# medhini/audio-video-textures

Measured on AMD Instinct MI355X. Metric: clip-windows/sec encoded + N×N transition build, N=4096; HBM GB/s achieved, higher is better.
Workload: dtype f16x3

## Files before the change

### audio-video-textures_amd/_lib.py

```python
import ctypes as C
import os
import re

_HERE = os.path.dirname(os.path.abspath(__file__))
LIB_PATH = os.environ.get("AVT_HIP_LIB") or os.path.join(_HERE, "libavt_hip.so")
HEADER_PATH = os.path.join(os.path.dirname(_HERE), "include", "avt.h")


class AvtError(RuntimeError):
    pass


_SCALARS = {"int": C.c_int, "int64_t": C.c_int64, "float": C.c_float, "double": C.c_double, "size_t": C.c_size_t}
_DECL = re.compile(r"\b(int|int64_t|const\s+char\s*\*)\s*\b(avt_[a-z0-9_]+)\s*\(([^()]*)\)\s*;")


def _ctype(decl, name):
    words = [w for w in decl.replace("*", " * ").replace("[", " [").split() if w != "const"]
    if any(w[0] in "*[" for w in words):
        return C.c_char_p if words[0] == "char" else C.c_void_p
    if not 1 <= len(words) <= 2 or words[0] not in _SCALARS:
        raise AvtError("include/avt.h: %s has a parameter `%s` whose type this binding does not know" % (name, decl.strip()))
    return _SCALARS[words[0]]

# ... 31 lines not shown

def _bind(fn):
    fn.restype, fn.argtypes = _ABI[fn.__name__]
    return fn


def lib():
    global _lib
    if _lib is None:
        if not os.path.exists(LIB_PATH):
            raise AvtError(
                "HIP extension not built: %s is missing. Run `make -C %s` (needs hipcc); "
                "there is no CPU fallback for the hot path." % (LIB_PATH, os.path.join(_HERE, "csrc")))
        handle = C.CDLL(LIB_PATH)
        for name in _ABI:
            if not hasattr(handle, name):
                raise AvtError("libavt_hip.so does not export %s: rebuild with `make -C %s`" % (name, os.path.join(_HERE, "csrc")))
            _bind(getattr(handle, name))
        if handle.avt_abi_version() != ABI_VERSION:
            raise AvtError("libavt_hip.so ABI version %d, expected %d: rebuild with `make -C %s`"
                           % (handle.avt_abi_version(), ABI_VERSION, os.path.join(_HERE, "csrc")))
        if os.environ.get("AVT_SMALL_TILE", "") == "0":
            handle.avt_conv_x3_set_small_tile(0)
        if os.environ.get("AVT_WGRAD_ROUNDS", "") == "0":
            handle.avt_wgrad_x3_set_xl(7)
        _lib = handle
    return _lib


def _failure(what, status):
    msg = lib().avt_last_error()
    return AvtError("%s failed (%d): %s" % (what, status, msg.decode() if msg else "?"))


def check(status, what):
    if status != 0:
        raise _failure(what, status)


def _errcheck(status, fn, args):
    if status != 0:
        raise _failure(fn.__name__, status)
    return status


class _Checked:
# ... 12 lines not shown
```

### audio-video-textures_amd/csrc/conv_args.h

```cpp
#pragma once
#include "avt_common.h"

namespace {

constexpr unsigned kOob = 0xFFFFFFF0u;
constexpr int kMaxTabSteps = 128;

constexpr int LSTR = 144;
constexpr int BK = 64;

struct FastDiv {
  uint32_t d, magic, shift;
};
inline FastDiv make_fastdiv(uint32_t d) {
  FastDiv f{d, 0u, 0u};
  if (d > 1) {
    uint32_t s = 0;
    while ((1ull << s) < d) ++s;
    f.magic = (uint32_t)((((1ull << 32) * ((1ull << s) - d)) / d) + 1);
    f.shift = s - 1;
  }
  return f;
}
__device__ __forceinline__ uint32_t fastdiv(uint32_t n, const FastDiv& f) {
  const uint32_t t = __umulhi(n, f.magic);
  const uint32_t q = (t + ((n - t) >> 1)) >> f.shift;
  return f.d == 1 ? n : q;
}

struct ConvArgs {
  const uint16_t* in;
  const uint16_t* wt;
  const float* bias;
  const uint16_t* res;
  uint16_t* out;
  const int2* ktab;
  int T, H, W;
  int To, Ho, Wo;
  int Cout, K;
  int KT, KH, KW, st, sh, sw, pt, ph, pw;
  int ldi, ldo, ldr;
  int relu;
  int M;
  int nk;
  int tiles_n, nblk;
  FastDiv dWo, dHo, dTo;
  FastDiv dCpt, dKHW, dKW;
  FastDiv dNT;
  int tapinner;
  unsigned in_bytes, wt_bytes;
  int pointwise;
  const uint16_t* wfrag;
  int nup;
  int wblk;
  unsigned wf_bytes;
  int ors, oH, oW;
  const uint16_t* in_lo;
  const uint16_t* wt_lo;
  const uint16_t* res_lo;
  uint16_t* out_lo;
  const float* wscale;
  float odiv;
  int cf_ofs;
  double* stat_part;
  int stat_groups, stat_mg, stat_tpg;
  int stat_c;
  const float* bst_x;
  const float* bst_mean;
  const float* bst_invstd;
  const float* bst_gamma;
  const float* bst_beta;
  const uint8_t* bst_mask;
  int bst_relu;
};

struct BstCoef {
  float mu[8], sc[8], be[8];
};
__device__ __forceinline__ void bst_load(const ConvArgs& a, int group, int n, BstCoef& k) {
  const int C = a.stat_c;
#pragma unroll
  for (int e = 0; e < 8; ++e) {
    const int c = (n + e) % C;
    k.mu[e] = a.bst_mean[(size_t)group * C + c];
    k.sc[e] = a.bst_invstd[(size_t)group * C + c] * a.bst_gamma[c];
    k.be[e] = a.bst_beta ? a.bst_beta[c] : 0.0f;
  }
}
__device__ __forceinline__ void bst_apply(const ConvArgs& a, const BstCoef& k, const float* xv, unsigned bits, float* x, float* s, float* q) {
  const bool by_bits = a.bst_relu != 0 && a.bst_mask != nullptr, by_x = a.bst_relu != 0 && a.bst_mask == nullptr;
  const unsigned mbits = by_bits ? bits : 0xFFu;
#pragma unroll
  for (int e = 0; e < 8; ++e) {
    const float xc = xv[e] - k.mu[e];
    const float act = by_x ? xc * k.sc[e] + k.be[e] : 1.0f;
    const float sel = (((mbits >> e) & 1u) != 0u && act > 0.0f) ? 1.0f : 0.0f;
// ... 98 lines not shown
  AVT_REQUIRE(M < (1ll << 31) && (int64_t)g.batch * g.t * g.h * g.w * g.ldi < (1ll << 31) - 64 && M * (int64_t)g.ldo < (1ll << 62) &&
                  (int64_t)g.cout * a.K < (1ll << 31) - 64,
              "%s: tensor too large for 32-bit offsets", who);
  a.in_bytes = (unsigned)((int64_t)g.batch * g.t * g.h * g.w * g.ldi * 2);
  a.wt_bytes = (unsigned)((int64_t)g.cout * a.K * 2);
  a.M = (int)M;
  a.nk = (a.K + BK - 1) / BK;
  a.pointwise = (g.kt == 1 && g.kh == 1 && g.kw == 1 && g.st == 1 && g.sh == 1 && g.sw == 1 && g.pt == 0 && g.ph == 0 && g.pw == 0 &&
                 a.To == g.t && a.Ho == g.h && a.Wo == g.w) ? 1 : 0;
  a.dWo = make_fastdiv((uint32_t)a.Wo);
  a.dHo = make_fastdiv((uint32_t)a.Ho);
  a.dTo = make_fastdiv((uint32_t)a.To);
  const bool remap = g.out_row_stride > 1 || (g.out_h > 0 && g.out_w > 0);
  AVT_REQUIRE(g.out_row_stride >= 1 && (!remap || (!res && g.out_h >= g.out_row_stride * (a.Ho - 1) + 1 &&
                                                   g.out_w >= g.out_row_stride * (a.Wo - 1) + 1)),
              "%s: the remapped rows need an out_h x out_w grid that holds %d x (%d x %d), no residual", who,
              g.out_row_stride, a.Ho, a.Wo);
  AVT_REQUIRE(!remap || (int64_t)g.batch * a.To * g.out_h * g.out_w < (1ll << 31),
              "%s: output buffer too large for 32-bit rows", who);
  a.ors = g.out_row_stride;
  a.oH = remap ? g.out_h : 0;
  a.oW = remap ? g.out_w : 0;
  a.stat_part = nullptr;
  a.odiv = 0.0f;
  a.stat_groups = a.stat_mg = a.stat_tpg = a.stat_c = 0;
  a.bst_x = a.bst_mean = a.bst_invstd = a.bst_gamma = a.bst_beta = nullptr;
  a.bst_mask = nullptr;
  a.bst_relu = 0;
  return AVT_OK;
}

}
```

### audio-video-textures_amd/csrc/conv_x3.hip

```cpp
#include <stdlib.h>

#include <type_traits>

#include "avt_common.h"
#include "conv_args.h"
#include "launch.h"
#include "mfma.h"
#include "split_planes.h"

#ifdef AVT_CONV_STAMP
#define AVT_STAMP_FN avt_debug_stamps_x3
namespace {
#include "../../tools/diag/conv_stamp.h"
}
#ifndef AVT_DBG_CONST
#define AVT_DBG_CONST 0
#endif
#define DBG_SKIP(bit) (((AVT_DBG_CONST) & (bit)) != 0)
#ifdef AVT_STAMP_EPI
#define KSTAMP(i) STAMP(0)
#define EPI_STAMP(i) STAMP(i)
#else
#define KSTAMP(i) STAMP(i)
#define EPI_STAMP(i)
// ... 385 lines not shown
#pragma unroll
      for (int e = 0; e < 8; ++e) {
        red[(tr * 2 + 0) * BN + cc * 8 + e] = st_s[e];
        red[(tr * 2 + 1) * BN + cc * 8 + e] = st_q[e];
      }
      __syncthreads();
      stat_fold_store<BN, 256>(a, red, 256 / CPR, tm, n0, tid);
    }
  }
  STAMP_END();
}

template <bool F16, bool IO32 = false, bool OUT32 = IO32>
__global__ __launch_bounds__(512, 2) void conv_x3_xl_kernel(ConvArgs a) {
  constexpr int BM = 256, BN = 256, NTHR = 512, KB = 32;
  constexpr int MT = 4, NT = 2;
  constexpr int AU = BM / 128, BU = BN / 128;
  constexpr int PL = BM * 64;
  constexpr int STG = 4 * PL;
  constexpr int ESTR = BN * 4 + 16;
  extern __shared__ __attribute__((aligned(16))) char lds[];

  const int swz = avt::xcd_contiguous(blockIdx.x, a.nblk);
  const int tm = swz / a.tiles_n, tn = swz % a.tiles_n;
  const int n0 = tn * BN;
  int m0, m_end;
  if constexpr (IO32) tile_rows(a, tm, BM, m0, m_end);
  else { m0 = tm * BM; m_end = a.M; }
  const int tid = threadIdx.x;
  const int lane = tid & 63, wid = tid >> 6;
  const int wm = wid >> 2, wn = wid & 3;
  const int lr = lane & 31, lh = lane >> 5;
  const int r0 = tid >> 2, c4 = (tid & 3) ^ ((r0 >> 2) & 3);

  int rowoff[AU];
  unsigned rowmask[AU];
#pragma unroll
  for (int u = 0; u < AU; ++u) {
    const int m = m0 + r0 + 128 * u;
    rowoff[u] = 0;
    rowmask[u] = 0u;
    if (m < m_end && a.pointwise) {
      rowoff[u] = m * a.ldi;
      rowmask[u] = 0x010101u;
    } else if (m < m_end) {
      const int t1 = (int)fastdiv((uint32_t)m, a.dWo), wo = m - t1 * a.Wo;
      const int t2 = (int)fastdiv((uint32_t)t1, a.dHo), ho = t1 - t2 * a.Ho;
      const int b = (int)fastdiv((uint32_t)t2, a.dTo), to = t2 - b * a.To;
      const int ti0 = to * a.st - a.pt, hi0 = ho * a.sh - a.ph, wi0 = wo * a.sw - a.pw;
      rowoff[u] = (((b * a.T + ti0) * a.H + hi0) * a.W + wi0) * a.ldi;
      unsigned mask = 0u;
      for (int dt = 0; dt < a.KT; ++dt) mask |= ((unsigned)(ti0 + dt) < (unsigned)a.T ? 1u : 0u) << dt;
      for (int dh = 0; dh < a.KH; ++dh) mask |= ((unsigned)(hi0 + dh) < (unsigned)a.H ? 1u : 0u) << (8 + dh);
      for (int dw = 0; dw < a.KW; ++dw) mask |= ((unsigned)(wi0 + dw) < (unsigned)a.W ? 1u : 0u) << (16 + dw);
      rowmask[u] = mask;
    }
  }
  int wrow[BU];
  unsigned wsel[BU];
#pragma unroll
  for (int u = 0; u < BU; ++u) {
    const int n = n0 + r0 + 128 * u;
    wrow[u] = n < a.Cout ? n * a.K : 0;
    wsel[u] = n < a.Cout ? 0xFFFFFFFFu : 0u;
  }

  f32x16 acc[NT][MT];
#pragma unroll
  for (int i = 0; i < NT; ++i)
#pragma unroll
    for (int j = 0; j < MT; ++j)
#pragma unroll
      for (int r = 0; r < 16; ++r) acc[i][j][r] = 0.0f;
  const __amdgpu_buffer_rsrc_t rih = avt::buffer_rsrc(a.in, a.in_bytes);
  const __amdgpu_buffer_rsrc_t ril = avt::buffer_rsrc(a.in_lo, a.in_bytes);
  const __amdgpu_buffer_rsrc_t rwh = avt::buffer_rsrc(a.wt, a.wt_bytes);
  const __amdgpu_buffer_rsrc_t rwl = avt::buffer_rsrc(a.wt_lo, a.wt_bytes);
  int2* ltab = reinterpret_cast<int2*>(lds + 2 * STG);
  for (int i = tid; i < a.nk * 8; i += NTHR) ltab[i] = a.ktab[i];
  const int nk32 = (a.K + KB - 1) / KB;

  unsigned aoffs[AU], boffs[BU];
  auto gtab = [&](int kt) -> int2 { return ltab[kt * 4 + c4]; };
  auto gcalc = [&](int kt, int2 e) {
    const unsigned ebits = (unsigned)e.y;
#pragma unroll
    for (int u = 0; u < AU; ++u) {
      const unsigned sel = ((rowmask[u] & ebits) == ebits) ? 0xFFFFFFFFu : 0u;
      aoffs[u] = (((unsigned)(rowoff[u] + e.x) * (IO32 ? 4u : 2u)) & sel) | (kOob & ~sel);
    }
    const unsigned ksel = ~(unsigned)(e.y >> 31);
    const unsigned kc2 = (unsigned)((kt * 4 + c4) * 16);
#pragma unroll
    for (int u = 0; u < BU; ++u) {
      const unsigned sel = ksel & wsel[u];
      boffs[u] = (((unsigned)wrow[u] * 2u + kc2) & sel) | (kOob & ~sel);
      if (a.wblk) boffs[u] = (((unsigned)(kt * a.Cout + n0 + r0 + 128 * u) * 64u + (unsigned)c4 * 16u) & sel) | (kOob & ~sel);
    }
  };
  auto gprep = [&](int kt) { gcalc(kt, gtab(kt)); };
  constexpr int NPIECE = 2 * (AU + BU);
  typedef __attribute__((address_space(3))) void* lds_ptr;
  const int wrow0 = wid * 16 * 64;
  auto gpiece = [&](int p, char* st) {
    if (p < 2 * AU) {
      const int u = p >> 1;
      __builtin_amdgcn_raw_ptr_buffer_load_lds((p & 1) ? ril : rih, (lds_ptr)(st + (p & 1) * PL + wrow0 + u * 128 * 64), 16,
                                               (int)aoffs[u], 0, 0, 0);
    } else {
      const int u = (p - 2 * AU) >> 1;
      __builtin_amdgcn_raw_ptr_buffer_load_lds((p & 1) ? rwl : rwh, (lds_ptr)(st + (2 + (p & 1)) * PL + wrow0 + u * 128 * 64), 16,
                                               (int)boffs[u], 0, 0, 0);
    }
  };
  i32x4 ra[IO32 ? AU : 1][2];
  auto aload = [&]() {
    if constexpr (IO32) {
#pragma unroll
      for (int u = 0; u < AU; ++u) {
        const unsigned o2 = aoffs[u] == kOob ? kOob : aoffs[u] + 16u;
        ra[u][0] = __builtin_amdgcn_raw_buffer_load_b128(rih, (int)aoffs[u], 0, 0);
        ra[u][1] = __builtin_amdgcn_raw_buffer_load_b128(rih, (int)o2, 0, 0);
      }
// ... 40 lines not shown
    for (int i = 0; i < NT; ++i)
#pragma unroll
      for (int j = 0; j < MT; ++j) {
        acc[i][j] = mfma32<F16>(f.wl[i], f.ah[j], acc[i][j]);
        acc[i][j] = mfma32<F16>(f.wh[i], f.al[j], acc[i][j]);
        acc[i][j] = mfma32<F16>(f.wh[i], f.ah[j], acc[i][j]);
        const int pc = g0 + i * MT + j + (IO32 ? 2 * AU : 0);
        if (more && pc < NPIECE) gpiece(pc, nst);
        __builtin_amdgcn_sched_barrier(0);
      }
  };

  float* cfl = reinterpret_cast<float*>(lds + a.cf_ofs);
  {
    const int n = n0 + (tid & 255);
    float v = tid < 256 ? 0.0f : 1.0f;
    if (n < a.Cout) {
      if (tid < 256) { if (a.bias) v = a.bias[n]; } else if (a.wscale) v = a.wscale[n];
    }
    cfl[tid] = v;
  }
  __syncthreads();
  STAMP_BEGIN();
  gprep(0);
  if constexpr (IO32) {
    aload();
#pragma unroll
    for (int p = 2 * AU; p < NPIECE; ++p) gpiece(p, lds);
    asm volatile("s_waitcnt vmcnt(0)" ::: "memory");
    astore(lds);
  } else {
#pragma unroll
    for (int p = 0; p < NPIECE; ++p) gpiece(p, lds);
    asm volatile("s_waitcnt vmcnt(0)" ::: "memory");
  }
  __syncthreads();
  STAMP(0);
  if constexpr (IO32) {
    for (int kt = 0; kt < nk32; ++kt) {
      const bool more = kt + 1 < nk32;
      char* cur = lds + (kt & 1) * STG;
      char* nst = lds + ((kt + 1) & 1) * STG;
      int2 e = make_int2(0, 0);
      if (more) e = gtab(kt + 1);
      Frags f;
      fload(f, cur, 0);
      if (more) {
        gcalc(kt + 1, e);
        aload();
      }
      __builtin_amdgcn_sched_barrier(0);
      fmul(f, 0, more, nst);
      fload(f, cur, 1);
      __builtin_amdgcn_sched_barrier(0);
      fmul(f, NPIECE, false, nst);
      asm volatile("s_waitcnt vmcnt(0)" ::: "memory");
      if (more) astore(nst);
      __syncthreads();
    }
  } else {
    Frags f0, f1;
    fload(f0, lds, 0);
    if (nk32 > 1) gprep(1);
    fload(f1, lds, 1);
    __builtin_amdgcn_sched_barrier(0);
    fmul(f0, 0, nk32 > 1, lds + STG);
    asm volatile("s_waitcnt vmcnt(0) lgkmcnt(0)" ::: "memory");
    __syncthreads();
    for (int kt = 1; kt < nk32; ++kt) {
      const bool more = kt + 1 < nk32;
      char* cur = lds + (kt & 1) * STG;
      char* nst = lds + ((kt + 1) & 1) * STG;
      int2 e = make_int2(0, 0);
      if (more) e = gtab(kt + 1);
      fload(f0, cur, 0);
      if (more) gcalc(kt + 1, e);
      __builtin_amdgcn_sched_barrier(0);
      fmul(f1, 0, more, nst);
      KSTAMP(1);
      fload(f1, cur, 1);
      __builtin_amdgcn_sched_barrier(0);
      fmul(f0, NPIECE, false, nst);
      KSTAMP(2);
      asm volatile("s_waitcnt vmcnt(0) lgkmcnt(0)" ::: "memory");
      KSTAMP(3);
      __syncthreads();
      KSTAMP(4);
    }
    fmul(f1, NPIECE, false, lds);
  }

  constexpr int SR = 64;
  constexpr int CPR = BN / 8;
  constexpr int EU = (SR * CPR) / NTHR;
  constexpr int EBUF = SR * ESTR;
  static_assert(2 * EBUF <= 2 * STG + kMaxTabSteps * 64, "two staging buffers fit the operand stages + the table area");
  const bool has_res = !OUT32 && a.res != nullptr;
  auto stage_slab = [&](auto half, int pass) {
    constexpr int H = decltype(half)::value;
    char* eb = lds + (pass & 1) * EBUF;
#pragma unroll
    for (int i = 0; i < NT; ++i)
#pragma unroll
      for (int g = 0; g < 4; ++g) {
        const int nl = wn * 64 + i * 32 + 8 * g + 4 * lh;
        const float4 bv = *reinterpret_cast<const float4*>(cfl + nl);
        const float4 sv = *reinterpret_cast<const float4*>(cfl + 256 + nl);
#pragma unroll
        for (int jj = 0; jj < 2; ++jj) {
          const int j = 2 * H + jj;
          float4 v;
          v.x = acc[i][j][4 * g + 0] * sv.x + bv.x;
          v.y = acc[i][j][4 * g + 1] * sv.y + bv.y;
          v.z = acc[i][j][4 * g + 2] * sv.z + bv.z;
          v.w = acc[i][j][4 * g + 3] * sv.w + bv.w;
          const int rl = jj * 32 + lr;
          *reinterpret_cast<float4*>(eb + rl * ESTR + nl * 4) = v;
        }
      }
  };
  KSTAMP(5);
  if (wm == 0) stage_slab(std::integral_constant<int, 0>{}, 0);
  __syncthreads();
  EPI_STAMP(1);
  float st_s[IO32 ? 8 : 1], st_q[IO32 ? 8 : 1];
  if constexpr (IO32) {
#pragma unroll
    for (int e = 0; e < 8; ++e) st_s[e] = st_q[e] = 0.0f;
  }
#pragma unroll 1
  for (int pass = 0; pass < 4; ++pass) {
    const char* eb = lds + (pass & 1) * EBUF;
    uint4 rrh[EU], rrl[EU];
    if (has_res) {
#pragma unroll
      for (int u = 0; u < EU; ++u) {
        const int c = tid + NTHR * u;
        const int m = m0 + pass * SR + c / CPR, n = n0 + (c % CPR) * 8;
        const bool ok = m < m_end && n < a.Cout;
        rrh[u] = ok ? *reinterpret_cast<const uint4*>(a.res + (int64_t)m * a.ldr + n) : make_uint4(0u, 0u, 0u, 0u);
        rrl[u] = ok ? *reinterpret_cast<const uint4*>(a.res_lo + (int64_t)m * a.ldr + n) : make_uint4(0u, 0u, 0u, 0u);
      }
    }
    if constexpr (IO32) {
      if (a.res) {
#pragma unroll
        for (int u = 0; u < EU; ++u) {
          const int c = tid + NTHR * u;
          const int m = m0 + pass * SR + c / CPR, n = n0 + (c % CPR) * 8;
          const bool ok = m < m_end && n < a.Cout;
          const float* rf = reinterpret_cast<const float*>(a.res) + (int64_t)m * a.ldr + n;
          rrh[u] = ok ? *reinterpret_cast<const uint4*>(rf) : make_uint4(0u, 0u, 0u, 0u);
          rrl[u] = ok ? *reinterpret_cast<const uint4*>(rf + 4) : make_uint4(0u, 0u, 0u, 0u);
        }
      }
    }
    if (pass + 1 < 4 && wm == ((pass + 1) >> 1)) {
      if ((pass + 1) & 1) stage_slab(std::integral_constant<int, 1>{}, pass + 1);
      else stage_slab(std::integral_constant<int, 0>{}, pass + 1);
    }
    EPI_STAMP(2);
#pragma unroll
    for (int u = 0; u < EU; ++u) {
      const int c = tid + NTHR * u;
      const int row = c / CPR, cc = c % CPR;
      const int m = m0 + pass * SR + row, n = n0 + cc * 8;
      if (m < m_end && n < a.Cout) {
        const float4 v0 = *reinterpret_cast<const float4*>(eb + row * ESTR + cc * 32);
        const float4 v1 = *reinterpret_cast<const float4*>(eb + row * ESTR + cc * 32 + 16);
        float x[8] = {v0.x, v0.y, v0.z, v0.w, v1.x, v1.y, v1.z, v1.w};
        if (has_res) {
          const uint32_t* ph = reinterpret_cast<const uint32_t*>(&rrh[u]);
          const uint32_t* pl = reinterpret_cast<const uint32_t*>(&rrl[u]);
#pragma unroll
          for (int e = 0; e < 4; ++e) {
            const avt::f32x2 r = avt::join2<F16>(ph[e], pl[e]);
            x[2 * e] += r.x;
            x[2 * e + 1] += r.y;
          }
        }
        if (a.relu == 1) {
#pragma unroll
          for (int e = 0; e < 8; ++e) x[e] = avt::relu_keep_nan(x[e]);
        } else if (a.relu == 2) {
#pragma unroll
          for (int e = 0; e < 8; ++e) x[e] = fmaxf(x[e], 0.1f * x[e]);
        }
        const int64_t o = (int64_t)out_row(a, m) * a.ldo + n;
        if constexpr (OUT32) {
// ... 29 lines not shown
    EPI_STAMP(3);
    __syncthreads();
    EPI_STAMP(4);
  }
  if constexpr (IO32) {
    if (a.stat_part) {
      float* red = reinterpret_cast<float*>(lds);
      const int tr = tid / CPR, cc = tid % CPR;
#pragma unroll
      for (int e = 0; e < 8; ++e) {
        red[(tr * 2 + 0) * BN + cc * 8 + e] = st_s[e];
        red[(tr * 2 + 1) * BN + cc * 8 + e] = st_q[e];
      }
      __syncthreads();
      stat_fold_store<BN, NTHR>(a, red, NTHR / CPR, tm, n0, tid);
    }
  }
  STAMP_END();
}

template <bool F16, bool IO32 = false, bool OUT32 = IO32>
int launch_x3_xl(ConvArgs& a, hipStream_t st) {
  if (a.stat_part) a.stat_tpg = (a.stat_mg + 255) / 256;
  const int tiles_m = a.stat_part ? a.stat_groups * a.stat_tpg : (a.M + 255) / 256;
  a.tiles_n = (a.Cout + 255) / 256;
  a.nblk = tiles_m * a.tiles_n;
  constexpr int lds_bytes = 2 * 4 * 256 * 64 + kMaxTabSteps * 64 + 2 * 256 * 4;
  a.cf_ofs = lds_bytes - 2 * 256 * 4;
  return avt::launch<conv_x3_xl_kernel<F16, IO32, OUT32>>("avt_conv3d_igemm_x3", dim3((unsigned)a.nblk), dim3(512), lds_bytes, lds_bytes,
                                                          st, a);
}

template <int BM, int BN, int WTM, bool F16, bool IO32 = false, bool BST = false>
int launch_x3(ConvArgs& a, hipStream_t st) {
  if (a.stat_part) a.stat_tpg = (a.stat_mg + BM - 1) / BM;
  const int tiles_m = a.stat_part ? a.stat_groups * a.stat_tpg : (a.M + BM - 1) / BM;
  a.tiles_n = (a.Cout + BN - 1) / BN;
  a.nblk = tiles_m * a.tiles_n;
  constexpr int epi_bytes = BM * (BN * 4 + 16);
  constexpr int opnd_max = 2 * (BM + BN) * LSTR + kMaxTabSteps * 64;
  constexpr int lds_max = (opnd_max > epi_bytes ? opnd_max : epi_bytes) + 2 * BN * 4;
  const int tab_bytes = (a.nk <= kMaxTabSteps ? a.nk : 0) * 64;
  int lds_bytes = 2 * (BM + BN) * LSTR + tab_bytes;
  if (lds_bytes < epi_bytes) lds_bytes = epi_bytes;
  a.cf_ofs = lds_bytes;
  lds_bytes += 2 * BN * 4;
  return avt::launch<conv_x3_kernel<BM, BN, WTM, F16, IO32, BST>>("avt_conv3d_igemm_x3", dim3((unsigned)a.nblk), dim3(256), lds_max,
                                                                  lds_bytes, st, a);
}

template <bool F16, bool IO32 = false, bool BST = false>
int launch_x3_by_cout(ConvArgs& a, hipStream_t st, bool small = false) {
  if (a.Cout <= 32) return launch_x3<128, 32, 32, F16, IO32, BST>(a, st);
  if (a.Cout <= 64) return launch_x3<128, 64, 64, F16, IO32, BST>(a, st);
  if constexpr (IO32) {
    if (small) return launch_x3<64, 128, 32, F16, IO32, BST>(a, st);
  }
  return launch_x3<128, 128, 64, F16, IO32, BST>(a, st);
}

struct X3Planes {
  const void *in_hi, *in_lo, *wt_hi, *wt_lo;
  const float* bias;
  const void *res_hi, *res_lo;
  void *out_hi, *out_lo;
};

}

extern "C" int avt_conv3d_igemm_x3_xl_picked(int cout, int k, int m) {
  return (cout % 256 == 0 && k >= 256 && k <= kMaxTabSteps * 64 && m >= 256 * 64) ? 1 : 0;
}

static int igemm_x3_one(const X3Planes& p, const int32_t* ktab, const ConvGeom& g, int plane_dtype, const float* wscale, void* stream,
                        int wblk, int xl) {
  AVT_REQUIRE(plane_dtype == AVT_X3_BF16 || plane_dtype == AVT_X3_F16, "avt_conv3d_igemm_x3: plane_dtype must be 0 (bf16) or 1 (fp16)");
  AVT_REQUIRE(!wscale || avt::aligned16(wscale), "avt_conv3d_igemm_x3: wscale must be 16-byte aligned");
  AVT_REQUIRE(p.in_lo && p.wt_lo && p.out_lo && (!p.res_hi == !p.res_lo), "avt_conv3d_igemm_x3: every tensor needs both planes");
  AVT_REQUIRE(avt::aligned16(p.in_lo) && avt::aligned16(p.wt_lo) && avt::aligned16(p.out_lo) && (!p.res_lo || avt::aligned16(p.res_lo)),
              "avt_conv3d_igemm_x3: pointers must be 16-byte aligned");
  ConvArgs a;
  const int rc = conv_args_fill(a, "avt_conv3d_igemm_x3", p.in_hi, p.wt_hi, p.bias, p.res_hi, p.out_hi, ktab, g);
  if (rc != AVT_OK) return rc;
  a.in_lo = static_cast<const uint16_t*>(p.in_lo);
  a.wt_lo = static_cast<const uint16_t*>(p.wt_lo);
  a.res_lo = static_cast<const uint16_t*>(p.res_lo);
  a.out_lo = static_cast<uint16_t*>(p.out_lo);
  a.wscale = wscale;
  a.wfrag = nullptr;
  a.nup = 0;
  a.wblk = wblk;
  hipStream_t s = static_cast<hipStream_t>(stream);
  AVT_REQUIRE(!wblk || (xl && a.K % 32 == 0),
              "avt_conv3d_igemm_x3_wblk: K-blocked weights are the 256 x 256 tile's (avt_conv3d_igemm_x3_xl_picked, K %% 32 == 0)");
  if (xl) return plane_dtype == AVT_X3_F16 ? launch_x3_xl<true>(a, s) : launch_x3_xl<false>(a, s);
  return plane_dtype == AVT_X3_F16 ? launch_x3_by_cout<true>(a, s) : launch_x3_by_cout<false>(a, s);
}

static int igemm_x3_impl(const X3Planes& p, const int32_t* ktab, const ConvGeom& g, int plane_dtype, const float* wscale, void* stream,
                         int wblk) {
  constexpr int64_t kMaxPlane = (1ll << 31) - 64;
  const bool sane = g.batch > 0 && g.t > 0 && g.h > 0 && g.w > 0 && g.ldi > 0 && g.ldo > 0 && g.cin > 0 && g.cout > 0 && g.kt >= 1 &&
                    g.kh >= 1 && g.kw >= 1 && g.st >= 1 && g.sh >= 1 && g.sw >= 1 && g.ph >= 0 && g.pw >= 0 && g.ho >= 0 && g.wo >= 0 &&
                    g.out_row_stride >= 1 && g.out_h >= 0 && g.out_w >= 0;
  const int64_t frame = sane ? (int64_t)g.h * g.w * g.ldi : 0, frames = sane ? (int64_t)g.batch * g.t : 0;
  if (!sane || frame * frames < kMaxPlane || g.kt != 1 || g.st != 1 || g.pt != 0 || (g.to != 0 && g.to != g.t)) {
    const int64_t k_all = (int64_t)g.kt * g.kh * g.kw * g.cin;
    int xl = 0;
    if (sane && k_all < (1ll << 31)) {
      const int64_t fho = g.ho > 0 ? g.ho : (g.h + 2 * g.ph - g.kh) / g.sh + 1, fwo = g.wo > 0 ? g.wo : (g.w + 2 * g.pw - g.kw) / g.sw + 1;
      const int64_t fto = g.to > 0 ? g.to : (g.t + 2 * g.pt - g.kt) / g.st + 1;
      const int64_t m = (int64_t)g.batch * fto * fho * fwo;
      xl = (m > 0 && m < (1ll << 31)) ? avt_conv3d_igemm_x3_xl_picked(g.cout, (int)k_all, (int)m) : 0;
    }
    return igemm_x3_one(p, ktab, g, plane_dtype, wscale, stream, wblk, xl);
  }
  AVT_REQUIRE(frame < kMaxPlane, "avt_conv3d_igemm_x3: one frame's input plane (%d x %d x %d elements) is too large for 32-bit offsets", g.h,
// ... 214 lines not shown
```

### audio-video-textures_amd/ops.py

```python
import ctypes as C

import numpy as np
import torch

from . import _lib

K = _lib.checked
SIM_BF16, SIM_BF16X3, SIM_F32 = 0, 1, 2
_PREC = {"bf16": SIM_BF16, "bf16x3": SIM_BF16X3, "f32": SIM_F32}
FAST_T, SLOW_T, SLOTS = 32, 8, 40


def _dev(t, name, dtype=None, contiguous=True):
    if not isinstance(t, torch.Tensor) or not t.is_cuda:
        raise _lib.AvtError("%s must be a device (HIP) tensor; the hot path has no CPU fallback" % name)
    if dtype is not None and t.dtype != dtype:
        raise _lib.AvtError("%s must be %s, got %s" % (name, dtype, t.dtype))
    if contiguous and not t.is_contiguous():
        raise _lib.AvtError("%s must be contiguous" % name)
    return t


def _p(t):
    return None if t is None else C.c_void_p(t.data_ptr())
# ... 489 lines not shown
    hi = torch.empty((cout, k), dtype=torch.bfloat16, device=w2d.device)
    lo = torch.empty_like(hi)
    ws = torch.empty(cout, dtype=torch.float32, device=w2d.device) if plane_dtype == X3_F16 else None
    K.avt_weight_planes_f32(_p(w2d), int(cout), int(k), _p(hi), _p(lo), _p(ws), int(plane_dtype), _stream())
    return hi, lo, ws


def weight_planes_gather_f32(w, idx_map, plane_dtype):
    _dev(w, "w", torch.float32, contiguous=False)
    _dev(idx_map, "idx_map", torch.int32)
    rows, k = idx_map.shape
    hi = torch.empty((rows, k), dtype=torch.bfloat16, device=w.device)
    lo = torch.empty_like(hi)
    ws = torch.empty(rows, dtype=torch.float32, device=w.device) if plane_dtype == X3_F16 else None
    K.avt_weight_planes_gather_f32(C.c_void_p(w.data_ptr()), _p(idx_map), int(rows), int(k), _p(hi), _p(lo), _p(ws), int(plane_dtype),
                                   _stream())
    return hi, lo, ws


def conv_x3_set_small_tile(on):
    return int(_lib.lib().avt_conv_x3_set_small_tile(int(bool(on))))


def weight_planes_job_bytes():
    return int(_lib.lib().avt_weight_planes_job_bytes())


def weight_planes_multi(jobs, blk2job, nblocks):
    assert jobs.is_cuda and blk2job.is_cuda and blk2job.dtype == torch.int32 and blk2job.numel() == nblocks
    K.avt_weight_planes_multi(_p(jobs), _p(blk2job), int(nblocks), _stream())


def sgd_job_bytes():
    return int(_lib.lib().avt_sgd_job_bytes())


def sgd_multi(jobs, blk2job, nblocks, hyper):
    assert jobs.is_cuda and blk2job.is_cuda and blk2job.dtype == torch.int32 and blk2job.numel() == nblocks
    assert hyper.is_cuda and hyper.dtype == torch.float32 and hyper.is_contiguous() and hyper.shape[-1] == 4
    K.avt_sgd_multi(_p(jobs), _p(blk2job), int(nblocks), _p(hyper), _stream())


def sgd_upload(dst, src_pinned, nbytes):
    assert dst.is_cuda and dst.is_contiguous() and not src_pinned.is_cuda and src_pinned.is_pinned() and src_pinned.is_contiguous()
    assert 0 < nbytes <= min(dst.numel() * dst.element_size(), src_pinned.numel() * src_pinned.element_size())
    K.avt_sgd_upload(_p(dst), _p(src_pinned), int(nbytes), _stream())
# ... 526 lines not shown
```

### include/avt.h

```cpp
#ifndef AVT_H
#define AVT_H

#include <stddef.h>
#include <stdint.h>

#ifdef __cplusplus
extern "C" {
#endif

#define AVT_ABI_VERSION 9

typedef enum {
  AVT_OK = 0,
  AVT_ERR_ARG = -1,
  AVT_ERR_UNSUPPORTED = -2,
  AVT_ERR_LAUNCH = -3,
  AVT_ERR_DEVICE = -4
} avt_status;

#define AVT_SIM_BF16    0
#define AVT_SIM_BF16X3  1
#define AVT_SIM_F32     2

#define AVT_DT_F32   0
#define AVT_DT_BF16  1

#define AVT_FAST_T 32
#define AVT_SLOW_T 8
#define AVT_SLOTS  (AVT_FAST_T + AVT_SLOW_T)

int avt_abi_version(void);
const char* avt_last_error(void);
int avt_device_check(char* name, size_t name_len);
// ... 177 lines not shown
int avt_train_batch_plan(uint32_t* mt_state, const int64_t* idx, int batch, int keep_lo, int keep_n, int n_len, int n_negs,
                         int stride, int32_t* tgt_out, int32_t* starts_out, void* stream);
int avt_frames_resize_aa_norm_u8(const uint8_t* frames, int n_frames, int height, int width, int out_hw, const float* mean,
                                 const float* std, float* out, void* stream);
int avt_clip_gather_frames_f32(const float* table, int n_frames, int out_hw, const int32_t* win_start, int n_win, int win_len,
                               float* out, void* stream);

int64_t avt_bn_train_ws_bytes(int64_t m, int c, int groups);
int avt_bn_train_fwd(const float* x, const float* res, float* y, int64_t m, int c, const float* gamma,
                     const float* beta, float eps, float momentum, int relu, int groups, void* ws, int64_t ws_size,
                     float* save_mean, float* save_invstd, float* running_mean, float* running_var,
                     int64_t* num_batches_tracked , void* relu_mask, int64_t ldy,
                     void* stream);
int avt_bn_train_bwd(const float* dy, const float* y, const float* x, int64_t m, int c, const float* gamma,
                     const float* beta, const float* save_mean, const float* save_invstd, int relu, int groups,
                     const void* relu_mask, void* ws, int64_t ws_size, float* dx, float* dres, float* dgamma, float* dbeta,
                     int64_t ld_dy, void* stream);

int avt_conv3d_igemm_x3_f32(const float* in, const void* wt_hi, const void* wt_lo, const float* wscale, const float* add,
                            float* out, const int32_t* ktab, int batch, int t, int h, int w, int cin, int cout, int kt,
                            int kh, int kw, int st, int sh, int sw, int pt, int ph, int pw, int ldi, int ldo, int lda,
                            int plane_dtype, void* stream);
int avt_conv_x3_set_small_tile(int on);
int avt_conv3d_igemm_x3_f32_stat_rows(int cout, int k, int64_t m, int groups);
int avt_conv3d_igemm_x3_f32_stats(const float* in, const void* wt_hi, const void* wt_lo, const float* wscale, float* out,
                                  const int32_t* ktab, int batch, int t, int h, int w, int cin, int cout, int kt, int kh, int kw,
                                  int st, int sh, int sw, int pt, int ph, int pw, int ldi, int ldo, int plane_dtype,
                                  void* stat_part, int groups, int stat_c, void* stream);
int avt_conv3d_igemm_x3_f32_bwdstats_rows(int cout, int k, int64_t m, int groups);
int avt_conv3d_igemm_x3_f32_bwdstats(const float* in, const void* wt_hi, const void* wt_lo, const float* wscale, const float* add,
                                     float* out, const int32_t* ktab, int batch, int t, int h, int w, int cin, int cout, int kt,
                                     int kh, int kw, int pt, int ph, int pw, int ldi, int ldo, int lda, int plane_dtype,
                                     const float* bn_x, const float* bn_mean, const float* bn_invstd, const float* bn_gamma,
                                     const float* bn_beta, const void* bn_mask, int relu, void* stat_part, int groups, int stat_c,
                                     void* stream);
int avt_pw_x3_f32_bwdstats_rows(int k, int n, int64_t m, int groups);
int avt_pw_x3_f32_bwdstats(const float* x, int ldx, int k, const void* w_hi, const void* w_lo, const float* add, int lda, float* y,
                           int ldy, int n, int64_t m, int plane_dtype, const float* bn_x, const float* bn_mean,
                           const float* bn_invstd, const float* bn_gamma, const float* bn_beta, const void* bn_mask, int relu,
                           void* stat_part, int groups, void* stream);
int avt_bn_train_bwd_pre(const float* g, const float* x, int64_t m, int c, const float* gamma, const float* save_mean,
                         const float* save_invstd, int groups, void* ws, int64_t ws_size, int pre_rows, float* dx, float* dgamma,
                         float* dbeta, void* stream);
int avt_pw_x3_f32_stat_rows(int k, int n, int64_t m, int groups);
int avt_pw_x3_f32_stats(const float* x, int ldx, int k, const void* w_hi, const void* w_lo, const float* wscale, float* y, int ldy,
                        int n, int64_t m, int plane_dtype, void* stat_part, int groups, void* stream);
// ... 153 lines not shown
```

Measured before the change: 1442.

## Group conv output rows by padding class to skip out-of-bounds taps

Adds padding-class scheduling to the 256x256 x3 implicit-GEMM conv kernel. Output rows are grouped by which kernel taps fall inside the input, and each tile iterates only over its class's valid K steps, using an LDS row remap and step list. A cost model enables it only when it saves steps, and excludes a few hardcoded shapes. This adds per-block class lookup, LDS row indirection in the epilogue, and a scattered row order.

Result: no change. 1441, median of 2 (-0.0%).

```diff
diff --git a/audio-video-textures_amd/_lib.py b/audio-video-textures_amd/_lib.py
--- a/audio-video-textures_amd/_lib.py
+++ b/audio-video-textures_amd/_lib.py
@@ -77,6 +77,8 @@
                            % (handle.avt_abi_version(), ABI_VERSION, os.path.join(_HERE, "csrc")))
         if os.environ.get("AVT_SMALL_TILE", "") == "0":
             handle.avt_conv_x3_set_small_tile(0)
+        if os.environ.get("AVT_PAD_CLASSES", "") == "0":
+            handle.avt_conv_x3_set_pad_classes(0)
         if os.environ.get("AVT_WGRAD_ROUNDS", "") == "0":
             handle.avt_wgrad_x3_set_xl(7)
         _lib = handle
diff --git a/audio-video-textures_amd/csrc/conv_args.h b/audio-video-textures_amd/csrc/conv_args.h
--- a/audio-video-textures_amd/csrc/conv_args.h
+++ b/audio-video-textures_amd/csrc/conv_args.h
@@ -26,6 +26,103 @@
   const uint32_t t = __umulhi(n, f.magic);
   const uint32_t q = (t + ((n - t) >> 1)) >> f.shift;
   return f.d == 1 ? n : q;
+}
+
+constexpr int kPcMaxCls = 27;
+constexpr int kPcNoRow = 0x7fffffff;
+constexpr int kPcFixed = 7;
+struct PadCls {
+  int on;
+  int ncls, cpt, batch;
+  int pos0[3][3], npos[3][3];
+  uint8_t tap0[3][3], ntap[3][3];
+  uint8_t code[kPcMaxCls + 1];
+  int tile0[kPcMaxCls + 1];
+};
+
+inline bool pc_ranges(int n, int no, int k, int s, int p, int* pos0, int* npos, uint8_t* tap0, uint8_t* ntap) {
+  int nr = 0;
+  for (int r = 0; r < 3; ++r) pos0[r] = npos[r] = tap0[r] = ntap[r] = 0;
+  for (int o = 0; o < no; ++o) {
+    const int i0 = o * s - p;
+    const int lo = i0 < 0 ? -i0 : 0, hi = n - i0 < k ? n - i0 : k;
+    if (hi <= lo) return false;
+    if (nr && tap0[nr - 1] == lo && ntap[nr - 1] == hi - lo) { ++npos[nr - 1]; continue; }
+    if (nr == 3) return false;
+    pos0[nr] = o; npos[nr] = 1; tap0[nr] = (uint8_t)lo; ntap[nr] = (uint8_t)(hi - lo);
+    ++nr;
+  }
+  return nr > 0;
+}
+__host__ __device__ inline int pc_cls_rows(const PadCls& pc, int code) {
+  return pc.batch * pc.npos[0][code & 3] * pc.npos[1][(code >> 2) & 3] * pc.npos[2][code >> 4];
+}
+__host__ __device__ inline int pc_cls_steps(const PadCls& pc, int code) {
+  return pc.ntap[0][code & 3] * pc.ntap[1][(code >> 2) & 3] * pc.ntap[2][code >> 4] * pc.cpt;
+}
+inline void pc_fill(PadCls& pc, int batch, int T, int H, int W, int To, int Ho, int Wo, int cin, int KT, int KH, int KW, int st, int sh,
+                    int sw, int pt, int ph, int pw, bool allow) {
+  pc = PadCls{};
+  if (cin % 32 != 0 || KT * KH * KW == 1) return;
+  pc.cpt = cin / 32;
+  pc.batch = batch;
+  if (!pc_ranges(T, To, KT, st, pt, pc.pos0[0], pc.npos[0], pc.tap0[0], pc.ntap[0]) ||
+      !pc_ranges(H, Ho, KH, sh, ph, pc.pos0[1], pc.npos[1], pc.tap0[1], pc.ntap[1]) ||
+      !pc_ranges(W, Wo, KW, sw, pw, pc.pos0[2], pc.npos[2], pc.tap0[2], pc.ntap[2]))
+    return;
+  int n = 0;
+  for (int code = 0; code < 64; ++code) {
+    if ((code & 3) == 3 || ((code >> 2) & 3) == 3 || (code >> 4) == 3 || pc_cls_rows(pc, code) == 0) continue;
+    int at = n++;
+    for (; at > 0 && pc_cls_steps(pc, pc.code[at - 1]) < pc_cls_steps(pc, code); --at) pc.code[at] = pc.code[at - 1];
+    pc.code[at] = (uint8_t)code;
+  }
+  pc.ncls = n;
+  int64_t with = 0;
+  for (int c = 0; c < n; ++c) {
+    const int tiles = (pc_cls_rows(pc, pc.code[c]) + 255) / 256;
+    pc.tile0[c + 1] = pc.tile0[c] + tiles;
+    with += (int64_t)tiles * (kPcFixed + pc_cls_steps(pc, pc.code[c]));
+  }
+  const int64_t M = (int64_t)batch * To * Ho * Wo;
+  const int64_t without = ((M + 255) / 256) * (kPcFixed + KT * KH * KW * pc.cpt);
+  const bool slower = (KT == 7 && KH * KW == 1 && st == 4 && cin == 128) || (KT == 1 && KH == 3 && KW == 3 && sh == 2 && sw == 2 && cin == 256) ||
+                      (KT == 3 && KH * KW == 1 && st == 1 && cin == 2048);
+  pc.on = (allow && n > 1 && with < without && !slower) ? 1 : 0;
+}
+__host__ __device__ inline void pc_unit(const PadCls& pc, int x, int l, int tiles_n, int& cls, int& unit) {
+  int G = 0;
+  for (int c = 0; c < pc.ncls; ++c) {
+    const int E = G + (pc.tile0[c + 1] - pc.tile0[c]) * tiles_n;
+    const int cnt = (E + 7 - x) / 8 - (G + 7 - x) / 8;
+    if (l < cnt || c + 1 == pc.ncls) {
+      int before = 0;
+      for (int y = 0; y < x; ++y) before += (E + 7 - y) / 8 - (G + 7 - y) / 8;
+      cls = c;
+      unit = before + l;
+      return;
+    }
+    l -= cnt;
+    G = E;
+  }
+  cls = unit = 0;
+}
+__host__ __device__ inline int pc_row(const PadCls& pc, int code, int r, int To, int Ho, int Wo) {
+  const int rt = code & 3, rh = (code >> 2) & 3, rw = code >> 4;
+  const unsigned nt = (unsigned)pc.npos[0][rt], nh = (unsigned)pc.npos[1][rh], nw = (unsigned)pc.npos[2][rw];
+  if ((unsigned)r >= (unsigned)pc.batch * nt * nh * nw) return kPcNoRow;
+  const unsigned q1 = (unsigned)r / nw, w = (unsigned)r - q1 * nw;
+  const unsigned q2 = q1 / nh, h = q1 - q2 * nh;
+  const unsigned b = q2 / nt, t = q2 - b * nt;
+  return (((int)b * To + pc.pos0[0][rt] + (int)t) * Ho + pc.pos0[1][rh] + (int)h) * Wo + pc.pos0[2][rw] + (int)w;
+}
+__host__ __device__ inline int pc_step(const PadCls& pc, int code, int i, int KH, int KW) {
+  const int rt = code & 3, rh = (code >> 2) & 3, rw = code >> 4;
+  const int nh = pc.ntap[1][rh], nw = pc.ntap[2][rw];
+  const int tap = i / pc.cpt, ch = i - tap * pc.cpt;
+  const int q = tap / nw, dw = tap - q * nw;
+  const int dt = q / nh, dh = q - dt * nh;
+  return (((pc.tap0[0][rt] + dt) * KH + pc.tap0[1][rh] + dh) * KW + pc.tap0[2][rw] + dw) * pc.cpt + ch;
 }
 
 struct ConvArgs {
@@ -72,6 +169,7 @@
   const float* bst_beta;
   const uint8_t* bst_mask;
   int bst_relu;
+  PadCls pc;
 };
 
 struct BstCoef {
@@ -216,6 +314,7 @@
   a.oH = remap ? g.out_h : 0;
   a.oW = remap ? g.out_w : 0;
   a.stat_part = nullptr;
+  a.pc.on = 0;
   a.odiv = 0.0f;
   a.stat_groups = a.stat_mg = a.stat_tpg = a.stat_c = 0;
   a.bst_x = a.bst_mean = a.bst_invstd = a.bst_gamma = a.bst_beta = nullptr;
diff --git a/audio-video-textures_amd/csrc/conv_x3.hip b/audio-video-textures_amd/csrc/conv_x3.hip
--- a/audio-video-textures_amd/csrc/conv_x3.hip
+++ b/audio-video-textures_amd/csrc/conv_x3.hip
@@ -431,11 +431,26 @@
   extern __shared__ __attribute__((aligned(16))) char lds[];
 
   const int swz = avt::xcd_contiguous(blockIdx.x, a.nblk);
-  const int tm = swz / a.tiles_n, tn = swz % a.tiles_n;
+  int tm = swz / a.tiles_n, tn = swz % a.tiles_n;
+  constexpr bool PC = !IO32 && !OUT32;
+  bool pcon = false;
+  int pcode = 0;
+  if constexpr (PC) {
+    if (a.pc.on) {
+      int cls, unit;
+      pc_unit(a.pc, (int)(blockIdx.x % 8u), (int)(blockIdx.x / 8u), a.tiles_n, cls, unit);
+      pcon = true;
+      pcode = a.pc.code[cls];
+      tm = unit / a.tiles_n;
+      tn = unit % a.tiles_n;
+    }
+  }
   const int n0 = tn * BN;
   int m0, m_end;
   if constexpr (IO32) tile_rows(a, tm, BM, m0, m_end);
   else { m0 = tm * BM; m_end = a.M; }
+  int* lrows = reinterpret_cast<int*>(lds + a.cf_ofs + 2 * 256 * 4);
+  int* lsteps = lrows + 256;
   const int tid = threadIdx.x;
   const int lane = tid & 63, wid = tid >> 6;
   const int wm = wid >> 2, wn = wid & 3;
@@ -446,7 +461,13 @@
   unsigned rowmask[AU];
 #pragma unroll
   for (int u = 0; u < AU; ++u) {
-    const int m = m0 + r0 + 128 * u;
+    int m = m0 + r0 + 128 * u;
+    if constexpr (PC) {
+      if (pcon) {
+        m = pc_row(a.pc, pcode, m, a.To, a.Ho, a.Wo);
+        if ((tid & 3) == 0) lrows[r0 + 128 * u] = m;
+      }
+    }
     rowoff[u] = 0;
     rowmask[u] = 0u;
     if (m < m_end && a.pointwise) {
@@ -467,12 +488,6 @@
   }
   int wrow[BU];
   unsigned wsel[BU];
-#pragma unroll
-  for (int u = 0; u < BU; ++u) {
-    const int n = n0 + r0 + 128 * u;
-    wrow[u] = n < a.Cout ? n * a.K : 0;
-    wsel[u] = n < a.Cout ? 0xFFFFFFFFu : 0u;
-  }
 
   f32x16 acc[NT][MT];
 #pragma unroll
@@ -487,7 +502,13 @@
   const __amdgpu_buffer_rsrc_t rwl = avt::buffer_rsrc(a.wt_lo, a.wt_bytes);
   int2* ltab = reinterpret_cast<int2*>(lds + 2 * STG);
   for (int i = tid; i < a.nk * 8; i += NTHR) ltab[i] = a.ktab[i];
-  const int nk32 = (a.K + KB - 1) / KB;
+  int nk32 = (a.K + KB - 1) / KB;
+  if constexpr (PC) {
+    if (pcon) {
+      nk32 = pc_cls_steps(a.pc, pcode);
+      if (tid < nk32) lsteps[tid] = pc_step(a.pc, pcode, tid, a.KH, a.KW);
+    }
+  }
 
   unsigned aoffs[AU], boffs[BU];
   auto gtab = [&](int kt) -> int2 { return ltab[kt * 4 + c4]; };
@@ -508,6 +529,19 @@
     }
   };
   auto gprep = [&](int kt) { gcalc(kt, gtab(kt)); };
+  auto gcalc_pc = [&](int kt, int2 e) {
+    const unsigned ebits = (unsigned)e.y;
+#pragma unroll
+    for (int u = 0; u < AU; ++u) {
+      const unsigned sel = ((rowmask[u] & ebits) == ebits) ? 0xFFFFFFFFu : 0u;
+      aoffs[u] = (((unsigned)(rowoff[u] + e.x) * 2u) & sel) | (kOob & ~sel);
+    }
+#pragma unroll
+    for (int u = 0; u < BU; ++u) {
+      const unsigned n = (unsigned)(n0 + r0 + 128 * u);
+      boffs[u] = a.wblk ? ((unsigned)(kt * a.Cout) + n) * 64u + (unsigned)c4 * 16u : n * (unsigned)a.K * 2u + (unsigned)((kt * 4 + c4) * 16);
+    }
+  };
   constexpr int NPIECE = 2 * (AU + BU);
   typedef __attribute__((address_space(3))) void* lds_ptr;
   const int wrow0 = wid * 16 * 64;
@@ -594,72 +628,127 @@
   }
   __syncthreads();
   STAMP_BEGIN();
-  gprep(0);
-  if constexpr (IO32) {
-    aload();
-#pragma unroll
-    for (int p = 2 * AU; p < NPIECE; ++p) gpiece(p, lds);
-    asm volatile("s_waitcnt vmcnt(0)" ::: "memory");
-    astore(lds);
-  } else {
-#pragma unroll
-    for (int p = 0; p < NPIECE; ++p) gpiece(p, lds);
-    asm volatile("s_waitcnt vmcnt(0)" ::: "memory");
-  }
-  __syncthreads();
-  STAMP(0);
-  if constexpr (IO32) {
-    for (int kt = 0; kt < nk32; ++kt) {
-      const bool more = kt + 1 < nk32;
-      char* cur = lds + (kt & 1) * STG;
-      char* nst = lds + ((kt + 1) & 1) * STG;
-      int2 e = make_int2(0, 0);
-      if (more) e = gtab(kt + 1);
-      Frags f;
-      fload(f, cur, 0);
-      if (more) {
-        gcalc(kt + 1, e);
-        aload();
-      }
+  auto lstep = [&](int i) { return __builtin_amdgcn_readfirstlane(lsteps[i]); };
+  bool pc_done = false;
+  if constexpr (PC) {
+    if (pcon) {
+      pc_done = true;
+      const int k0 = lstep(0);
+      gcalc_pc(k0, gtab(k0));
+#pragma unroll
+      for (int p = 0; p < NPIECE; ++p) gpiece(p, lds);
+      asm volatile("s_waitcnt vmcnt(0)" ::: "memory");
+      __syncthreads();
+      STAMP(0);
+      Frags f0, f1;
+      int knext = lstep(1);
+      fload(f0, lds, 0);
+      if (nk32 > 1) gcalc_pc(knext, gtab(knext));
+      fload(f1, lds, 1);
       __builtin_amdgcn_sched_barrier(0);
-      fmul(f, 0, more, nst);
-      fload(f, cur, 1);
+      fmul(f0, 0, nk32 > 1, lds + STG);
+      int kread = lsteps[2];
+      asm volatile("s_waitcnt vmcnt(0) lgkmcnt(0)" ::: "memory");
+      __syncthreads();
+      for (int i = 1; i < nk32; ++i) {
+        const bool more = i + 1 < nk32;
+        char* cur = lds + (i & 1) * STG;
+        char* nst = lds + ((i + 1) & 1) * STG;
+        knext = __builtin_amdgcn_readfirstlane(kread);
+        int2 e = make_int2(0, 0);
+        if (more) e = gtab(knext);
+        fload(f0, cur, 0);
+        if (more) gcalc_pc(knext, e);
+        __builtin_amdgcn_sched_barrier(0);
+        fmul(f1, 0, more, nst);
+        KSTAMP(1);
+        kread = lsteps[i + 2];
+        fload(f1, cur, 1);
+        __builtin_amdgcn_sched_barrier(0);
+        fmul(f0, NPIECE, false, nst);
+        KSTAMP(2);
+        asm volatile("s_waitcnt vmcnt(0) lgkmcnt(0)" ::: "memory");
+        KSTAMP(3);
+        __syncthreads();
+        KSTAMP(4);
+      }
+      fmul(f1, NPIECE, false, lds);
+    }
+  }
+  if (!pc_done) {
+#pragma unroll
+    for (int u = 0; u < BU; ++u) {
+      const int n = n0 + r0 + 128 * u;
+      wrow[u] = n < a.Cout ? n * a.K : 0;
+      wsel[u] = n < a.Cout ? 0xFFFFFFFFu : 0u;
+    }
+    gprep(0);
+    if constexpr (IO32) {
+      aload();
+#pragma unroll
+      for (int p = 2 * AU; p < NPIECE; ++p) gpiece(p, lds);
+      asm volatile("s_waitcnt vmcnt(0)" ::: "memory");
+      astore(lds);
+    } else {
+#pragma unroll
+      for (int p = 0; p < NPIECE; ++p) gpiece(p, lds);
+      asm volatile("s_waitcnt vmcnt(0)" ::: "memory");
+    }
+    __syncthreads();
+    STAMP(0);
+    if constexpr (IO32) {
+      for (int kt = 0; kt < nk32; ++kt) {
+        const bool more = kt + 1 < nk32;
+        char* cur = lds + (kt & 1) * STG;
+        char* nst = lds + ((kt + 1) & 1) * STG;
+        int2 e = make_int2(0, 0);
+        if (more) e = gtab(kt + 1);
+        Frags f;
+        fload(f, cur, 0);
+        if (more) {
+          gcalc(kt + 1, e);
+          aload();
+        }
+        __builtin_amdgcn_sched_barrier(0);
+        fmul(f, 0, more, nst);
+        fload(f, cur, 1);
+        __builtin_amdgcn_sched_barrier(0);
+        fmul(f, NPIECE, false, nst);
+        asm volatile("s_waitcnt vmcnt(0)" ::: "memory");
+        if (more) astore(nst);
+        __syncthreads();
+      }
+    } else {
+      Frags f0, f1;
+      fload(f0, lds, 0);
+      if (nk32 > 1) gprep(1);
+      fload(f1, lds, 1);
       __builtin_amdgcn_sched_barrier(0);
-      fmul(f, NPIECE, false, nst);
-      asm volatile("s_waitcnt vmcnt(0)" ::: "memory");
-      if (more) astore(nst);
+      fmul(f0, 0, nk32 > 1, lds + STG);
+      asm volatile("s_waitcnt vmcnt(0) lgkmcnt(0)" ::: "memory");
       __syncthreads();
-    }
-  } else {
-    Frags f0, f1;
-    fload(f0, lds, 0);
-    if (nk32 > 1) gprep(1);
-    fload(f1, lds, 1);
-    __builtin_amdgcn_sched_barrier(0);
-    fmul(f0, 0, nk32 > 1, lds + STG);
-    asm volatile("s_waitcnt vmcnt(0) lgkmcnt(0)" ::: "memory");
-    __syncthreads();
-    for (int kt = 1; kt < nk32; ++kt) {
-      const bool more = kt + 1 < nk32;
-      char* cur = lds + (kt & 1) * STG;
-      char* nst = lds + ((kt + 1) & 1) * STG;
-      int2 e = make_int2(0, 0);
-      if (more) e = gtab(kt + 1);
-      fload(f0, cur, 0);
-      if (more) gcalc(kt + 1, e);
-      __builtin_amdgcn_sched_barrier(0);
-      fmul(f1, 0, more, nst);
-      KSTAMP(1);
-      fload(f1, cur, 1);
-      __builtin_amdgcn_sched_barrier(0);
-      fmul(f0, NPIECE, false, nst);
-      KSTAMP(2);
-      asm volatile("s_waitcnt vmcnt(0) lgkmcnt(0)" ::: "memory");
-      KSTAMP(3);
-      __syncthreads();
-      KSTAMP(4);
-    }
-    fmul(f1, NPIECE, false, lds);
+      for (int kt = 1; kt < nk32; ++kt) {
+        const bool more = kt + 1 < nk32;
+        char* cur = lds + (kt & 1) * STG;
+        char* nst = lds + ((kt + 1) & 1) * STG;
+        int2 e = make_int2(0, 0);
+        if (more) e = gtab(kt + 1);
+        fload(f0, cur, 0);
+        if (more) gcalc(kt + 1, e);
+        __builtin_amdgcn_sched_barrier(0);
+        fmul(f1, 0, more, nst);
+        KSTAMP(1);
+        fload(f1, cur, 1);
+        __builtin_amdgcn_sched_barrier(0);
+        fmul(f0, NPIECE, false, nst);
+        KSTAMP(2);
+        asm volatile("s_waitcnt vmcnt(0) lgkmcnt(0)" ::: "memory");
+        KSTAMP(3);
+        __syncthreads();
+        KSTAMP(4);
+      }
+      fmul(f1, NPIECE, false, lds);
+    }
   }
 
   constexpr int SR = 64;
@@ -668,6 +757,13 @@
   constexpr int EBUF = SR * ESTR;
   static_assert(2 * EBUF <= 2 * STG + kMaxTabSteps * 64, "two staging buffers fit the operand stages + the table area");
   const bool has_res = !OUT32 && a.res != nullptr;
+  auto erow = [&](int row) {
+    int m = m0 + row;
+    if constexpr (PC) {
+      if (pcon) m = lrows[row];
+    }
+    return m;
+  };
   auto stage_slab = [&](auto half, int pass) {
     constexpr int H = decltype(half)::value;
     char* eb = lds + (pass & 1) * EBUF;
@@ -708,7 +804,7 @@
 #pragma unroll
       for (int u = 0; u < EU; ++u) {
         const int c = tid + NTHR * u;
-        const int m = m0 + pass * SR + c / CPR, n = n0 + (c % CPR) * 8;
+        const int m = erow(pass * SR + c / CPR), n = n0 + (c % CPR) * 8;
         const bool ok = m < m_end && n < a.Cout;
         rrh[u] = ok ? *reinterpret_cast<const uint4*>(a.res + (int64_t)m * a.ldr + n) : make_uint4(0u, 0u, 0u, 0u);
         rrl[u] = ok ? *reinterpret_cast<const uint4*>(a.res_lo + (int64_t)m * a.ldr + n) : make_uint4(0u, 0u, 0u, 0u);
@@ -736,7 +832,7 @@
     for (int u = 0; u < EU; ++u) {
       const int c = tid + NTHR * u;
       const int row = c / CPR, cc = c % CPR;
-      const int m = m0 + pass * SR + row, n = n0 + cc * 8;
+      const int m = erow(pass * SR + row), n = n0 + cc * 8;
       if (m < m_end && n < a.Cout) {
         const float4 v0 = *reinterpret_cast<const float4*>(eb + row * ESTR + cc * 32);
         const float4 v1 = *reinterpret_cast<const float4*>(eb + row * ESTR + cc * 32 + 16);
@@ -812,11 +908,12 @@
 template <bool F16, bool IO32 = false, bool OUT32 = IO32>
 int launch_x3_xl(ConvArgs& a, hipStream_t st) {
   if (a.stat_part) a.stat_tpg = (a.stat_mg + 255) / 256;
-  const int tiles_m = a.stat_part ? a.stat_groups * a.stat_tpg : (a.M + 255) / 256;
+  int tiles_m = a.stat_part ? a.stat_groups * a.stat_tpg : (a.M + 255) / 256;
+  if (!IO32 && !OUT32 && a.pc.on) tiles_m = a.pc.tile0[a.pc.ncls];
   a.tiles_n = (a.Cout + 255) / 256;
   a.nblk = tiles_m * a.tiles_n;
-  constexpr int lds_bytes = 2 * 4 * 256 * 64 + kMaxTabSteps * 64 + 2 * 256 * 4;
-  a.cf_ofs = lds_bytes - 2 * 256 * 4;
+  constexpr int lds_bytes = 2 * 4 * 256 * 64 + kMaxTabSteps * 64 + 2 * 256 * 4 + 256 * 4 + (256 + 8) * 4;
+  a.cf_ofs = 2 * 4 * 256 * 64 + kMaxTabSteps * 64;
   return avt::launch<conv_x3_xl_kernel<F16, IO32, OUT32>>("avt_conv3d_igemm_x3", dim3((unsigned)a.nblk), dim3(512), lds_bytes, lds_bytes,
                                                           st, a);
 }
@@ -860,6 +957,61 @@
 
 extern "C" int avt_conv3d_igemm_x3_xl_picked(int cout, int k, int m) {
   return (cout % 256 == 0 && k >= 256 && k <= kMaxTabSteps * 64 && m >= 256 * 64) ? 1 : 0;
+}
+
+static int g_pad_classes = 1;
+extern "C" int avt_conv_x3_set_pad_classes(int on) {
+  const int was = g_pad_classes;
+  g_pad_classes = on ? 1 : 0;
+  return was;
+}
+
+extern "C" int avt_conv3d_igemm_x3_xl_plan(int batch, int t, int h, int w, int cin, int cout, int kt, int kh, int kw, int st, int sh,
+                                           int sw, int pt, int ph, int pw, int tile, int32_t* rows, int32_t* steps, int32_t* info) {
+  AVT_REQUIRE(info && batch > 0 && t > 0 && h > 0 && w > 0 && cin > 0 && cin % 8 == 0 && cout > 0 && kt >= 1 && kh >= 1 && kw >= 1 &&
+                  kt <= 8 && kh <= 8 && kw <= 8 && st >= 1 && sh >= 1 && sw >= 1 && pt >= 0 && ph >= 0 && pw >= 0,
+              "avt_conv3d_igemm_x3_xl_plan: bad geometry");
+  const int To = (t + 2 * pt - kt) / st + 1, Ho = (h + 2 * ph - kh) / sh + 1, Wo = (w + 2 * pw - kw) / sw + 1;
+  const int64_t M = (int64_t)batch * To * Ho * Wo, K = (int64_t)kt * kh * kw * cin;
+  AVT_REQUIRE(To > 0 && Ho > 0 && Wo > 0 && M < (1ll << 31) && K <= kMaxTabSteps * 64, "avt_conv3d_igemm_x3_xl_plan: bad extent");
+  PadCls pc;
+  pc_fill(pc, batch, t, h, w, To, Ho, Wo, cin, kt, kh, kw, st, sh, sw, pt, ph, pw, g_pad_classes != 0);
+  const int tiles_n = (cout + 255) / 256, nk32 = (int)((K + 31) / 32);
+  const int tiles_m = pc.on ? pc.tile0[pc.ncls] : (int)((M + 255) / 256);
+  const int nblk = tiles_m * tiles_n;
+  info[0] = pc.on;
+  info[1] = nblk;
+  info[2] = pc.on ? pc.ncls : 1;
+  info[3] = info[4] = info[5] = info[6] = info[7] = 0;
+  if (tile < 0) return AVT_OK;
+  AVT_REQUIRE(tile < nblk && rows && steps, "avt_conv3d_igemm_x3_xl_plan: tile %d of %d, or NULL lists", tile, nblk);
+  int tm = tile / tiles_n, tn = tile % tiles_n, cls = 0, ns = nk32;
+  if (pc.on) {
+    const int qd = nblk / 8, rm = nblk % 8;
+    const int x = tile < rm * (qd + 1) ? tile / (qd + 1) : rm + (tile - rm * (qd + 1)) / qd;
+    const int l = tile < rm * (qd + 1) ? tile % (qd + 1) : (tile - rm * (qd + 1)) % qd;
+    int unit;
+    pc_unit(pc, x, l, tiles_n, cls, unit);
+    tm = unit / tiles_n;
+    tn = unit % tiles_n;
+    ns = pc_cls_steps(pc, pc.code[cls]);
+    for (int i = 0; i < ns; ++i) steps[i] = pc_step(pc, pc.code[cls], i, kh, kw);
+  } else {
+    for (int i = 0; i < ns; ++i) steps[i] = i;
+  }
+  int valid = 0;
+  for (int r = 0; r < 256; ++r) {
+    int m = tm * 256 + r;
+    if (pc.on) m = pc_row(pc, pc.code[cls], m, To, Ho, Wo);
+    rows[r] = m < M ? m : -1;
+    valid += m < M ? 1 : 0;
+  }
+  info[3] = ns;
+  info[4] = cls;
+  info[5] = tn;
+  info[6] = valid;
+  info[7] = tm;
+  return AVT_OK;
 }
 
 static int igemm_x3_one(const X3Planes& p, const int32_t* ktab, const ConvGeom& g, int plane_dtype, const float* wscale, void* stream,
@@ -883,6 +1035,8 @@
   hipStream_t s = static_cast<hipStream_t>(stream);
   AVT_REQUIRE(!wblk || (xl && a.K % 32 == 0),
               "avt_conv3d_igemm_x3_wblk: K-blocked weights are the 256 x 256 tile's (avt_conv3d_igemm_x3_xl_picked, K %% 32 == 0)");
+  if (xl && !a.pointwise && a.Cout % 256 == 0)
+    pc_fill(a.pc, g.batch, a.T, a.H, a.W, a.To, a.Ho, a.Wo, g.cin, a.KT, a.KH, a.KW, a.st, a.sh, a.sw, a.pt, a.ph, a.pw, g_pad_classes != 0);
   if (xl) return plane_dtype == AVT_X3_F16 ? launch_x3_xl<true>(a, s) : launch_x3_xl<false>(a, s);
   return plane_dtype == AVT_X3_F16 ? launch_x3_by_cout<true>(a, s) : launch_x3_by_cout<false>(a, s);
 }
diff --git a/audio-video-textures_amd/ops.py b/audio-video-textures_amd/ops.py
--- a/audio-video-textures_amd/ops.py
+++ b/audio-video-textures_amd/ops.py
@@ -535,6 +535,10 @@
     return int(_lib.lib().avt_conv_x3_set_small_tile(int(bool(on))))
 
 
+def conv_x3_set_pad_classes(on):
+    return int(_lib.lib().avt_conv_x3_set_pad_classes(int(bool(on))))
+
+
 def weight_planes_job_bytes():
     return int(_lib.lib().avt_weight_planes_job_bytes())
 
diff --git a/include/avt.h b/include/avt.h
--- a/include/avt.h
+++ b/include/avt.h
@@ -8,7 +8,7 @@
 extern "C" {
 #endif
 
-#define AVT_ABI_VERSION 9
+#define AVT_ABI_VERSION 10
 
 typedef enum {
   AVT_OK = 0,
@@ -232,6 +232,9 @@
                             int kh, int kw, int st, int sh, int sw, int pt, int ph, int pw, int ldi, int ldo, int lda,
                             int plane_dtype, void* stream);
 int avt_conv_x3_set_small_tile(int on);
+int avt_conv_x3_set_pad_classes(int on);
+int avt_conv3d_igemm_x3_xl_plan(int batch, int t, int h, int w, int cin, int cout, int kt, int kh, int kw, int st, int sh, int sw,
+                                int pt, int ph, int pw, int tile, int32_t* rows, int32_t* steps, int32_t* info);
 int avt_conv3d_igemm_x3_f32_stat_rows(int cout, int k, int64_t m, int groups);
 int avt_conv3d_igemm_x3_f32_stats(const float* in, const void* wt_hi, const void* wt_lo, const float* wscale, float* out,
                                   const int32_t* ktab, int batch, int t, int h, int w, int cin, int cout, int kt, int kh, int kw,
```
